# lsl036/STM-Multifrontal-QR-Factorization-Empowered-by-GCN

Hardware: AMD Instinct MI355X
Metric: numerical-factorization GFLOP/s (higher is better)
Workload: dtype f64; 1 GPU; xenon1_colamd_standin: m=49248 n=49248 nnz=1258432 fronts=686 flops/step=5.029e+11, ordering default (COLAMD: qrtest without an ordering argument) (stand-in for xenon1.mtx, absent from the reference checkout); inputs=values resident in HBM, factors left in HBM, parallelism=replica x1, levels=16, retries=0

## Files before the change

stm-multifrontal-qr-factorization-empowered-by-gcn_amd/csrc/stmmqr_kdev.h:

```cpp
#pragma once
#include <hip/hip_runtime.h>
#include <hip/hip_ext.h>
#include <stdint.h>
#include <stdlib.h>
#include "stmmqr_device.h"
#include "stmmqr_kernels.h"
#include "stmmqr_wave.h"
#include "stmmqr_devutil.h"

struct PanelShared {
    double red[16];
    int st_out[STM_NB];
    int dead[STM_NB];
    double nextss;
    int nextss_col;
    int stair[STM_NB];
    int diag[STM_NB];
    double tau[STM_NB];
    double G[STM_NB][STM_NB + 1];
    double T[STM_NB][STM_NB + 1];
    double part[8 * 32];
    double top[2][8];
    double rsum[2][64];
    double rsumB[5][64];
    double Ts[8][9];
    double gp[32];
};

#define NT 256
#define NW (NT / 64)
#define BN 32
#define RB 64
#define VS (RB + 2)
#define WS (BN + 1)

template <int NTH>
__device__ __forceinline__ double block_sum(double v, double *s_red)
{
    v = wave_sum(v);
    __syncthreads();
    if ((threadIdx.x & 63) == 0) s_red[threadIdx.x >> 6] = v;
    __syncthreads();
    double r = 0;
#pragma unroll
    for (int w = 0; w < NTH / 64; w++) r += s_red[w];
    return r;
}

__device__ __forceinline__ int block_incl_scan(int v, int *s_scan, int *total)
{
    const int lane = threadIdx.x & 63, wid = threadIdx.x >> 6;
    int x = v;
#pragma unroll
    for (int o = 1; o < 64; o <<= 1) {
        int y = __shfl_up(x, o, 64);
        if (lane >= o) x += y;
    }
    __syncthreads();
    if (lane == 63) s_scan[wid] = x;
    __syncthreads();
    int base = 0, tot = 0;
#pragma unroll
    for (int w = 0; w < NW; w++) {
        int sw = s_scan[w];
        if (w < wid) base += sw;
        tot += sw;
    }
    *total = tot;
    return x + base;
}

#define SLAB STM_UPD_SLAB
#define CK(x) do { hipError_t e_ = (x); if (e_ != hipSuccess) return (int)e_; } while (0)


struct UpdChunk { double v[8], c[8]; };
__device__ __forceinline__ void upd_chunk_load(UpdChunk &ck, const double *Vg, const double *Cg, long long ld, int i, int mp,
                                               int nbp, int nc, int lcg)
{
    const int ic = min(i, mp - 1);
#pragma unroll
    for (int q = 0; q < 8; q++) {
        const int col = lcg * 8 + q;
        ck.v[q] = Vg[ic + (long long)min(col, nbp - 1) * ld];
        ck.c[q] = Cg[ic + (long long)min(col, nc - 1) * ld];
    }
}
__device__ __forceinline__ void upd_chunk_to_lds(const UpdChunk &ck, int i, int mp, int nbp, int nc, const int *s_pd, int g1,
                                                 int lrow, int lcg, double *Vs, double *Cs, bool c_is_v = false, bool plain = false)
{
    if (plain) {
#pragma unroll
        for (int q = 0; q < 8; q++) {
            const int col = lcg * 8 + q;
            Vs[col * VS + lrow] = ck.v[q];
            Cs[col * VS + lrow] = c_is_v ? ck.v[q] : ck.c[q];
        }
        return;
    }
#pragma unroll
    for (int q = 0; q < 8; q++) {
        const int col = lcg * 8 + q;
        const int d = s_pd[col] - g1;
        const double v = (i < mp && col < nbp && i >= d) ? ((i == d) ? 1.0 : ck.v[q]) : 0.0;
        Vs[col * VS + lrow] = v;
        Cs[col * VS + lrow] = c_is_v ? v : ((i < mp && col < nc) ? ck.c[q] : 0.0);
    }
}

__device__ __forceinline__ void upd_chunk_v_to_lds(const UpdChunk &ck, int i, int mp, int nbp, const int *s_pd, int g1, int lrow,
                                                   int lcg, double *Vs, bool plain = false)
{
    if (plain) {
#pragma unroll
        for (int q = 0; q < 8; q++) Vs[(lcg * 8 + q) * VS + lrow] = ck.v[q];
        return;
    }
#pragma unroll
    for (int q = 0; q < 8; q++) {
        const int col = lcg * 8 + q;
        const int d = s_pd[col] - g1;
        Vs[col * VS + lrow] = (i < mp && col < nbp && i >= d) ? ((i == d) ? 1.0 : ck.v[q]) : 0.0;
    }
}
__device__ __forceinline__ int upd_plain_from(const int *s_pd, int g1, int lane)
{
    const int dm = wave_max_int(lane < STM_NB ? s_pd[lane] : -1);
    return dm >= STM_BIGROW ? STM_BIGROW : dm - g1;
}

__device__ __forceinline__ void dev_T_from_gram(double (*G)[STM_NB + 1], double (*T)[STM_NB + 1], const double *tau, int nc, int tid);

__device__ __forceinline__ d4 dev_w2_tile(const double *Tm, int sq, int sl, const double *W1, int wid, int lane)
{
    const int mi = wid >> 1, ni = wid & 1, l15 = lane & 15, l4 = lane >> 4;
    d4 acc = {0, 0, 0, 0};
    const int nk = mi ? STM_NB / 4 : STM_NB / 8;
#pragma unroll
    for (int kk = 0; kk < STM_NB / 4; kk++) {
        if (kk < nk) {
            const double a = Tm[(4 * kk + l4) * sq + (16 * mi + l15) * sl];
            const double b = W1[(4 * kk + l4) * WS + 16 * ni + l15];
            acc = __builtin_amdgcn_mfma_f64_16x16x4f64(a, b, acc, 0, 0, 0);
        }
    }
    return acc;
}

#define STM_UPD_LDS_DOUBLES (2 * BN * VS + STM_NB * WS)
static_assert(STM_UPD_LDS_DOUBLES == STM_UPD_LDS_HOST, "host sizing of the update kernels' LDS");
template <bool TN = false>
__device__ void dev_update_block(double *F, long long ld, int g1, int mp, int k1, int nbp, const int *diag,
                                 const double *T, int c0, int nc, double *lds, const double *tau = nullptr,
                                 double *Tout = nullptr, double *Tkeep = nullptr)
{
    if (nbp <= 0 || mp <= 0 || nc <= 0) return;
    const int tid = (int)threadIdx.x, lane = tid & 63, wid = tid >> 6;
    const int l15 = lane & 15, l4 = lane >> 4;

    double *Vs = lds;
    double *Cs = Vs + STM_NB * VS;
    double *Ws = Cs + BN * VS;
    __shared__ int s_pd[STM_NB];

    __syncthreads();
    if (tid < STM_NB) s_pd[tid] = (tid < nbp) ? diag[tid] : STM_BIGROW;
    __syncthreads();

    const int lrow = tid & 63, lcg = tid >> 6;
    const double *Vg = F + g1 + (long long)k1 * ld;
    double *Cg = F + g1 + (long long)c0 * ld;

    const int mi = wid >> 1, ni = wid & 1;
    const bool build_t = (tau != nullptr);
    d4 acc = {0, 0, 0, 0}, tot = {0, 0, 0, 0}, gacc = {0, 0, 0, 0}, gtot = {0, 0, 0, 0};
    UpdChunk ck;
    upd_chunk_load(ck, Vg, Cg, ld, lrow, mp, nbp, nc, lcg);
    for (int r0 = 0; r0 < mp; r0 += RB) {
        const int i = r0 + lrow;
        upd_chunk_to_lds(ck, i, mp, nbp, nc, s_pd, g1, lrow, lcg, Vs, Cs);
        __syncthreads();
        if (r0 + RB < mp) upd_chunk_load(ck, Vg, Cg, ld, i + RB, mp, nbp, nc, lcg);
#pragma unroll
        for (int kk = 0; kk < RB / 4; kk++) {
            const double a = Vs[(16 * mi + l15) * VS + 4 * kk + l4];
            const double b = Cs[(16 * ni + l15) * VS + 4 * kk + l4];
            acc = __builtin_amdgcn_mfma_f64_16x16x4f64(a, b, acc, 0, 0, 0);
            if (build_t) {
                const double bv = Vs[(16 * ni + l15) * VS + 4 * kk + l4];
                gacc = __builtin_amdgcn_mfma_f64_16x16x4f64(a, bv, gacc, 0, 0, 0);
            }
        }
        if ((r0 + RB) % STM_UPD_SLAB == 0 || r0 + RB >= mp) {
#pragma unroll
            for (int r = 0; r < 4; r++) { tot[r] += acc[r]; acc[r] = 0; gtot[r] += gacc[r]; gacc[r] = 0; }
        }
        __syncthreads();
    }
#pragma unroll
    for (int r = 0; r < 4; r++) Ws[(16 * mi + l4 + 4 * r) * WS + 16 * ni + l15] = tot[r];
    double *s_Tm = Cs;
    if (build_t) {
        double (*Gm)[STM_NB + 1] = reinterpret_cast<double (*)[STM_NB + 1]>(Vs);
        __shared__ double s_tau_u[STM_NB];
#pragma unroll
        for (int r = 0; r < 4; r++) Gm[16 * mi + l4 + 4 * r][16 * ni + l15] = gtot[r];
        if (tid < STM_NB) s_tau_u[tid] = (tid < nbp) ? tau[tid] : 0.0;
        __syncthreads();
        dev_T_from_gram(Gm, reinterpret_cast<double (*)[STM_NB + 1]>(s_Tm), s_tau_u, nbp, tid);
        if (Tout || Tkeep)
            for (int e = tid; e < STM_NB * STM_NB; e += (int)blockDim.x) {
                const int a = e % STM_NB, b = e / STM_NB;
                const double tv = (a <= b && a < nbp && b < nbp) ? s_Tm[a * WS + b] : 0.0;
                if (Tout) Tout[e] = tv;
                if (Tkeep) Tkeep[e] = tv;
            }
    }
    __syncthreads();

    {
        const int l = tid & 31, cg = tid >> 5;
        double w2[4] = {0, 0, 0, 0};
        if (TN) {
            for (int q = l; q < nbp; q++) {
                const double tq = build_t ? s_Tm[l * WS + q] : T[l + q * STM_NB];
#pragma unroll
                for (int x = 0; x < 4; x++) w2[x] += tq * Ws[q * WS + cg * 4 + x];
            }
            __syncthreads();
#pragma unroll
            for (int x = 0; x < 4; x++) Ws[l * WS + cg * 4 + x] = w2[x];
        } else {
            d4 t2 = {0, 0, 0, 0};
            if (wid < 4) t2 = build_t ? dev_w2_tile(s_Tm, WS, 1, Ws, wid, lane) : dev_w2_tile(T, 1, STM_NB, Ws, wid, lane);
            __syncthreads();
            if (wid < 4) {
#pragma unroll
                for (int r = 0; r < 4; r++) Ws[(16 * mi + l4 + 4 * r) * WS + 16 * ni + l15] = t2[r];
            }
        }
    }
    __syncthreads();

    upd_chunk_load(ck, Vg, Cg, ld, lrow, mp, nbp, nc, lcg);
    for (int r0 = 0; r0 < mp; r0 += RB) {
        const int i = r0 + lrow;
        upd_chunk_to_lds(ck, i, mp, nbp, nc, s_pd, g1, lrow, lcg, Vs, Cs);
        __syncthreads();
        if (r0 + RB < mp) upd_chunk_load(ck, Vg, Cg, ld, i + RB, mp, nbp, nc, lcg);
        d4 u0 = {0, 0, 0, 0}, u1 = {0, 0, 0, 0};
#pragma unroll
        for (int kk = 0; kk < STM_NB / 4; kk++) {
            const double a = Vs[(4 * kk + l4) * VS + 16 * wid + l15];
            const double b0 = Ws[(4 * kk + l4) * WS + l15];
            const double b1 = Ws[(4 * kk + l4) * WS + 16 + l15];
            u0 = __builtin_amdgcn_mfma_f64_16x16x4f64(a, b0, u0, 0, 0, 0);
            u1 = __builtin_amdgcn_mfma_f64_16x16x4f64(a, b1, u1, 0, 0, 0);
        }
#pragma unroll
        for (int r = 0; r < 4; r++) {
            const int row = 16 * wid + l4 + 4 * r;
            Cs[l15 * VS + row] -= u0[r];
            Cs[(16 + l15) * VS + row] -= u1[r];
        }
        __syncthreads();
        if (i < mp) {
#pragma unroll
            for (int q = 0; q < 8; q++) {
                const int col = lcg * 8 + q;
                if (col < nc) Cg[i + col * ld] = Cs[col * VS + lrow];
            }
        }
        __syncthreads();
    }
}

template <int h>
__device__ __forceinline__ void dev_T_merge(double (*G)[STM_NB + 1], double (*T)[STM_NB + 1], int tid)
{
    const int pr = tid / (h * h), ij = tid % (h * h), i = ij / h, j = ij % h;
    const int A0 = 2 * h * pr, B0 = A0 + h;
// ... 142 lines not shown
```

stm-multifrontal-qr-factorization-empowered-by-gcn_amd/csrc/stmmqr_riders.h:

```cpp
#pragma once
#include "stmmqr_kdev.h"


#define STM_PC_LDS_DOUBLES (STM_NB * WS + 4 * BN * VS)
__device__ __forceinline__ void dev_upd_c_h2(const DevCtx &c, const int *__restrict__ flist, const int *__restrict__ plist, int cb0,
                                             const double *Wp, const long long *__restrict__ wpoff, int fi, int cb, int sl0,
                                             int rspw, double *dyn_lds, int *s_pd)
{
    const int f = flist[fi], p = plist[fi];
    const FrontSym s = c.fs[f];
    if (p >= s.npanels) return;
    const PanelDesc *pd = &c.fnum[f].pd[STM_PDI(p)];
    const int g1 = pd->pg1, mp = pd->pt - pd->pg1, nbp = pd->pnb;
    const int nslf = stm_upd_nsl(s);
    const int c0 = pd->pc0 + (cb0 + cb * (1 + c.cbskip)) * BN;
    const int sl = sl0 * rspw, spw = rspw;
    if (nbp <= 0 || mp <= 0 || c0 >= s.fn || sl * SLAB >= mp) return;
    const int nc = min(BN, s.fn - c0);
    const long long ld = s.ld;
    const int half = threadIdx.x >> 8, tid = threadIdx.x & 255, lane = tid & 63, wid = tid >> 6, l15 = lane & 15, l4 = lane >> 4;
    double *Ws = dyn_lds, *Vs = Ws + STM_NB * WS + half * (2 * BN * VS), *Cs = Vs + BN * VS;
    double *s_W1 = dyn_lds + STM_NB * WS, *s_T = s_W1 + BN * VS;
    if (threadIdx.x < STM_NB) s_pd[threadIdx.x] = ((int)threadIdx.x < nbp) ? pd->pdiag[threadIdx.x] : STM_BIGROW;
    const double *Vg = c.Farena + s.foff + g1 + (long long)pd->pk1 * ld;
    double *Cg = c.Farena + s.foff + g1 + (long long)c0 * ld;
    const int lrow = tid & 63, lcg = tid >> 6;
    const int rbeg = sl * SLAB, rend = min(mp, (sl + spw) * SLAB);
    int r0 = rbeg + half * RB;
    UpdChunk ck0, ck1;
    upd_chunk_load(ck0, Vg, Cg, ld, r0 + lrow, mp, nbp, nc, lcg);
    upd_chunk_load(ck1, Vg, Cg, ld, r0 + 2 * RB + lrow, mp, nbp, nc, lcg);
    {
        const double *W0 = Wp + wpoff[fi] + ((long long)cb * nslf) * (STM_NB * BN);
        const double *T = c.Tws + (long long)STM_TSLOT(c.tslot[f], p) * STM_NB * STM_NB;
        for (int e = threadIdx.x; e < STM_NB * BN; e += 2 * NT) {
            const double v = W0[e];
            s_W1[(e / BN) * WS + (e % BN)] = v;
            s_T[(e / STM_NB) * WS + (e % STM_NB)] = T[e];
        }
        __syncthreads();
        d4 w2 = {0, 0, 0, 0};
        if (half == 0) w2 = dev_w2_tile(s_T, 1, WS, s_W1, wid, lane);
        __syncthreads();
        if (half == 0) {
#pragma unroll
            for (int r = 0; r < 4; r++) Ws[(16 * (wid >> 1) + l4 + 4 * r) * WS + 16 * (wid & 1) + l15] = w2[r];
        }
    }
    const int pfrom = upd_plain_from(s_pd, g1, lane);
    const int nch = (rend - rbeg + RB - 1) / RB, trips = (nch + 1) / 2;
    auto trip = [&](UpdChunk &ck) {
        const bool valid = r0 < rend;
        const int i = r0 + lrow;
        double cc[8];
#pragma unroll
        for (int q = 0; q < 8; q++) cc[q] = ck.c[q];
        upd_chunk_v_to_lds(ck, i, mp, nbp, s_pd, g1, lrow, lcg, Vs, valid && r0 > pfrom && r0 + RB <= mp);
        __syncthreads();
        if (r0 + 4 * RB < rend) upd_chunk_load(ck, Vg, Cg, ld, i + 4 * RB, mp, nbp, nc, lcg);
        d4 u0 = {0, 0, 0, 0}, u1 = {0, 0, 0, 0};
#pragma unroll
        for (int kk = 0; kk < STM_NB / 4; kk++) {
            const double a = Vs[(4 * kk + l4) * VS + 16 * wid + l15];
            const double b0 = Ws[(4 * kk + l4) * WS + l15];
            const double b1 = Ws[(4 * kk + l4) * WS + 16 + l15];
            u0 = __builtin_amdgcn_mfma_f64_16x16x4f64(a, b0, u0, 0, 0, 0);
            u1 = __builtin_amdgcn_mfma_f64_16x16x4f64(a, b1, u1, 0, 0, 0);
        }
#pragma unroll
        for (int r = 0; r < 4; r++) {
            const int row = 16 * wid + l4 + 4 * r;
            Cs[l15 * VS + row] = u0[r];
            Cs[(16 + l15) * VS + row] = u1[r];
        }
        __syncthreads();
        if (valid && i < mp) {
#pragma unroll
            for (int q = 0; q < 8; q++) {
                const int col = lcg * 8 + q;
                if (col < nc) Cg[i + col * ld] = cc[q] - Cs[col * VS + lrow];
            }
        }
        r0 += 2 * RB;
    };
    for (int j = 0; j < trips; j += 2) {
        trip(ck0);
        if (j + 1 < trips) trip(ck1);
    }
}
```

stm-multifrontal-qr-factorization-empowered-by-gcn_amd/csrc/stmmqr_update.hip:

```cpp
#include <hip/hip_ext.h>
#include "stmmqr_kdev.h"


__global__ __launch_bounds__(NT) void k_update(DevCtx c, const int *__restrict__ flist, const int *__restrict__ plist, int cb0)
{
    extern __shared__ double dyn_lds[];
    const int f = flist[blockIdx.y];
    const int p = plist[blockIdx.y];
    const FrontSym s = c.fs[f];
    if (p >= s.npanels) return;
    const PanelDesc *pd = &c.fnum[f].pd[STM_PDI(p)];
    const int cbg = cb0 + (int)blockIdx.x * (1 + c.cbskip);
    const int c0 = pd->pc0 + cbg * BN;
    if (c0 >= s.fn) return;
    double *Tw = c.Tws + (long long)STM_TSLOT(c.tslot[f], p) * STM_NB * STM_NB;
    if (pd->t_deferred) {
        const bool first = (cbg == 0) || (c.cbskip > 0 && blockIdx.x == 0);
        dev_update_block(c.Farena + s.foff, s.ld, pd->pg1, pd->pt - pd->pg1, pd->pk1, pd->pnb, pd->pdiag, nullptr, c0,
                         min(BN, s.fn - c0), dyn_lds, c.Tau + s.rp + pd->pk1, first ? Tw : nullptr,
                         (first && c.Tall) ? c.Tall + (long long)(s.tpan + p) * STM_NB * STM_NB : nullptr);
        return;
    }
    dev_update_block(c.Farena + s.foff, s.ld, pd->pg1, pd->pt - pd->pg1, pd->pk1, pd->pnb, pd->pdiag, Tw, c0,
                     min(BN, s.fn - c0), dyn_lds);
// ... 304 lines not shown
            }
            __syncthreads();
        }
    }
    const int nsl = (mp + SLAB - 1) / SLAB;
    const int gslot = (c.ypoff && c.ypoff[f] >= 0) ? min(ncbf, c.sweep) : ncbf;
    double *Wslot = Wp + wpoff[fi] + ((long long)(gram ? gslot : cb) * nslf) * (STM_NB * BN);
    double *W = Wslot + (long long)sl * (STM_NB * BN);
#pragma unroll
    for (int r = 0; r < 4; r++) st_agent(&W[(16 * mi + l4 + 4 * r) * BN + 16 * ni + l15], acc[r]);
    asm volatile("s_waitcnt vmcnt(0)" ::: "memory");
    __syncthreads();
    double *Tslot = c.Tws + (long long)STM_TSLOT(c.tslot[f], p) * STM_NB * STM_NB;
    if (gram) {
        if (tid == 0) {
            s_ticket = __hip_atomic_fetch_add(&num->gcnt, 1, __ATOMIC_RELAXED, __HIP_MEMORY_SCOPE_AGENT);
            if (s_ticket == nsl - 1) {
                __builtin_amdgcn_fence(__ATOMIC_ACQUIRE, "agent");
                asm volatile("s_waitcnt vmcnt(0)" ::: "memory");
                __hip_atomic_store(&num->gcnt, 0, __ATOMIC_RELAXED, __HIP_MEMORY_SCOPE_AGENT);
            }
        }
        __syncthreads();
        if (s_ticket != nsl - 1) return;
        double *s_G = Vs;
        __shared__ double s_tau[STM_NB];
        if (tid < STM_NB) s_tau[tid] = (tid < nbp) ? c.Tau[s.rp + pd->pk1 + tid] : 0.0;
        for (int e = tid; e < STM_NB * BN; e += NT) {
            const double gsum = stm_ordered_sum<true>(Wslot + e, STM_NB * BN, nsl);
            s_G[(e / BN) * WS + (e % BN)] = gsum;
        }
        __syncthreads();
        double *Tkeep = c.Tall ? c.Tall + (long long)(s.tpan + p) * STM_NB * STM_NB : nullptr;
        double (*s_Tb)[STM_NB + 1] = reinterpret_cast<double (*)[STM_NB + 1]>(Cs);
        dev_T_from_gram(reinterpret_cast<double (*)[STM_NB + 1]>(s_G), s_Tb, s_tau, nbp, threadIdx.x);
        for (int e = tid; e < STM_NB * STM_NB; e += NT) {
            const int a = e % STM_NB, b = e / STM_NB;
            const double tv = (a <= b && a < nbp && b < nbp) ? s_Tb[a][b] : 0.0;
            st_agent(&Tslot[e], tv);
            if (Tkeep) Tkeep[e] = tv;
        }
        asm volatile("s_waitcnt vmcnt(0)" ::: "memory");
        __syncthreads();
        if (tid == 0) st_agent(&num->tready, epoch);
        return;
    }
    int *cnt = wcnt + wpoff[fi] / (STM_NB * BN) + cb;
    int *flag = wflag + wpoff[fi] / (STM_NB * BN) + cb;
    bool last = (nsl == 1);
    if (nsl > 1) {
        if (tid == 0) {
            s_ticket = __hip_atomic_fetch_add(cnt, 1, __ATOMIC_RELAXED, __HIP_MEMORY_SCOPE_AGENT);
            if (s_ticket == nsl - 1) {
                __builtin_amdgcn_fence(__ATOMIC_ACQUIRE, "agent");
                asm volatile("s_waitcnt vmcnt(0)" ::: "memory");
                __hip_atomic_store(cnt, 0, __ATOMIC_RELAXED, __HIP_MEMORY_SCOPE_AGENT);
            }
        }
        __syncthreads();
        last = (s_ticket == nsl - 1);
    }
    double *s_W1 = Vs, *s_T = Cs;
    if (last) {
        if (pd->t_deferred && !stm_wait_ge(&num->tready, epoch, c.abort, &s_ok)) { if (tid == 0) STM_SET_PERR(c, num); return; }
        for (int e = tid; e < STM_NB * BN; e += NT) {
            const double v = stm_ordered_sum<true>(Wslot + e, STM_NB * BN, nsl);
            s_W1[(e / BN) * WS + (e % BN)] = v;
            s_T[(e / STM_NB) * WS + (e % STM_NB)] = ld_agent(&Tslot[e]);
        }
        __syncthreads();
        const d4 w2 = dev_w2_tile(s_T, 1, WS, s_W1, wid, lane);
#pragma unroll
        for (int r = 0; r < 4; r++) Ws[(16 * (wid >> 1) + l4 + 4 * r) * WS + 16 * (wid & 1) + l15] = w2[r];
        if (nsl > 1) {
#pragma unroll
            for (int r = 0; r < 4; r++) st_agent(&Wslot[(16 * (wid >> 1) + l4 + 4 * r) * BN + 16 * (wid & 1) + l15], w2[r]);
            asm volatile("s_waitcnt vmcnt(0)" ::: "memory");
            __syncthreads();
            if (tid == 0) st_agent(flag, epoch);
        } else
            __syncthreads();
    } else {
        if (!stm_wait_ge(flag, epoch, c.abort, &s_ok)) { if (tid == 0) STM_SET_PERR(c, num); return; }
        for (int e = tid; e < STM_NB * BN; e += NT) Ws[(e / BN) * WS + (e % BN)] = ld_agent(&Wslot[e]);
        __syncthreads();
    }
#pragma unroll
    for (int q = 0; q < SLAB / RB; q++) {
        const int r0 = r00 + q * RB;
        if (r0 < rend) {
            const int i = r0 + lrow;
            upd_chunk_to_lds(ck[q], i, mp, nbp, nc, s_pd, g1, lrow, lcg, Vs, Cs);
            __syncthreads();
            d4 u0 = {0, 0, 0, 0}, u1 = {0, 0, 0, 0};
#pragma unroll
            for (int kk = 0; kk < STM_NB / 4; kk++) {
                const double a = Vs[(4 * kk + l4) * VS + 16 * wid + l15];
                const double b0 = Ws[(4 * kk + l4) * WS + l15];
                const double b1 = Ws[(4 * kk + l4) * WS + 16 + l15];
                u0 = __builtin_amdgcn_mfma_f64_16x16x4f64(a, b0, u0, 0, 0, 0);
                u1 = __builtin_amdgcn_mfma_f64_16x16x4f64(a, b1, u1, 0, 0, 0);
            }
#pragma unroll
            for (int r = 0; r < 4; r++) {
                const int row = 16 * wid + l4 + 4 * r;
                Cs[l15 * VS + row] -= u0[r];
                Cs[(16 + l15) * VS + row] -= u1[r];
            }
            __syncthreads();
            if (i < mp) {
#pragma unroll
                for (int qq = 0; qq < 8; qq++) {
                    const int col = lcg * 8 + qq;
                    if (col < nc) Cg[i + col * ld] = Cs[col * VS + lrow];
                }
            }
            __syncthreads();
        }
    }
}

__global__ __launch_bounds__(NT, 2) void k_upd_f(DevCtx c, const int *__restrict__ flist, const int *__restrict__ plist, int cb0,
                                              int with_gram, double *Wp, const long long *__restrict__ wpoff, int *wcnt,
                                              int *wflag, int epoch)
{
    extern __shared__ double dyn_lds[];
    dev_k_upd_f(c, flist, plist, cb0, with_gram, Wp, wpoff, wcnt, wflag, epoch, blockIdx.x, blockIdx.y, blockIdx.z, dyn_lds);
}

__device__ __forceinline__ void dev_k_upd_b0(const DevCtx &c, const int *__restrict__ flist, const int *__restrict__ plist, double *Wp,
                                             const long long *__restrict__ wpoff, int *wcnt, int *wflag, int epoch, int sl, int fi,
                                             double *dyn_lds)
{
    __shared__ int s_pd[STM_NB];
    __shared__ int s_ticket, s_ok;
    __shared__ double s_tau[STM_NB];
    const bool tl = (c.dbg & 32768) && c.dbgbuf && threadIdx.x == 0 && sl == 0;
    unsigned long long tl0 = tl ? wall_clock64() : 0;
#define B0TL(k) do { if (tl) { const unsigned long long t1 = wall_clock64(); atomicAdd(&c.dbgbuf[48 + (k)], t1 - tl0); tl0 = t1; } } while (0)
    const int f = flist[fi], p = plist[fi];
    const FrontSym s = c.fs[f];
    if (p >= s.npanels) return;
    FrontNum *num = &c.fnum[f];
    const PanelDesc *pd = &num->pd[STM_PDI(p)];
    const int g1 = pd->pg1, mp = pd->pt - pd->pg1, nbp = pd->pnb;
    const int ncbf = stm_upd_ncb(s, p), nslf = stm_upd_nsl(s);
    if (ncbf <= 0) return;
    const int c0 = pd->pc0;
    if (nbp <= 0 || mp <= 0 || c0 >= s.fn || sl * SLAB >= mp) return;
    const bool deferred = pd->t_deferred != 0;
    const int nc = min(BN, s.fn - c0);
    const long long ld = s.ld;
    const int tid = threadIdx.x, lane = tid & 63, wid = tid >> 6, l15 = lane & 15, l4 = lane >> 4;
    const int lrow = tid & 63, lcg = tid >> 6;
    double *Vs = dyn_lds, *Cs = Vs + STM_NB * VS, *Ws = Cs + BN * VS;
    if (tid < STM_NB) {
        s_pd[tid] = (tid < nbp) ? pd->pdiag[tid] : STM_BIGROW;
        s_tau[tid] = (tid < nbp) ? c.Tau[s.rp + pd->pk1 + tid] : 0.0;
    }
    const double *Vg = c.Farena + s.foff + g1 + (long long)pd->pk1 * ld;
    double *Cg = c.Farena + s.foff + g1 + (long long)c0 * ld;
    const int r00 = sl * SLAB, rend = min(mp, (sl + 1) * SLAB);
    UpdChunk ck[SLAB / RB];
#pragma unroll
    for (int q = 0; q < SLAB / RB; q++) upd_chunk_load(ck[q], Vg, Cg, ld, r00 + q * RB + lrow, mp, nbp, nc, lcg);
    const int nsl = (mp + SLAB - 1) / SLAB;
    const int gslot = (c.ypoff && c.ypoff[f] >= 0) ? min(ncbf, c.sweep) : ncbf;
    double *Wslot = Wp + wpoff[fi];
    double *Gslot = Wp + wpoff[fi] + ((long long)gslot * nslf) * (STM_NB * BN);
    double *Tslot = c.Tws + (long long)STM_TSLOT(c.tslot[f], p) * STM_NB * STM_NB;
    __syncthreads();
    B0TL(0);
    const int mi = wid >> 1, ni = wid & 1;
    d4 acc = {0, 0, 0, 0}, accg = {0, 0, 0, 0};
#pragma unroll
    for (int q = 0; q < SLAB / RB; q++) {
        const int r0 = r00 + q * RB;
        if (r0 < rend) {
            upd_chunk_to_lds(ck[q], r0 + lrow, mp, nbp, nc, s_pd, g1, lrow, lcg, Vs, Cs);
            __syncthreads();
#pragma unroll
            for (int kk = 0; kk < RB / 4; kk++) {
                const double a = Vs[(16 * mi + l15) * VS + 4 * kk + l4];
                const double b = Cs[(16 * ni + l15) * VS + 4 * kk + l4];
                acc = __builtin_amdgcn_mfma_f64_16x16x4f64(a, b, acc, 0, 0, 0);
            }
            if (deferred) {
#pragma unroll
                for (int kk = 0; kk < RB / 4; kk++) {
                    const double a = Vs[(16 * mi + l15) * VS + 4 * kk + l4];
                    const double b = Vs[(16 * ni + l15) * VS + 4 * kk + l4];
                    accg = __builtin_amdgcn_mfma_f64_16x16x4f64(a, b, accg, 0, 0, 0);
                }
            }
            __syncthreads();
        }
    }
    double *s_G = Vs, *s_W1 = Vs + STM_NB * WS, *s_T = Cs;
    B0TL(1);
    bool last = true;
    if (nsl > 1) {
        double *W = Wslot + (long long)sl * (STM_NB * BN), *G = Gslot + (long long)sl * (STM_NB * BN);
#pragma unroll
        for (int r = 0; r < 4; r++) st_agent(&W[(16 * mi + l4 + 4 * r) * BN + 16 * ni + l15], acc[r]);
        if (deferred) {
#pragma unroll
            for (int r = 0; r < 4; r++) st_agent(&G[(16 * mi + l4 + 4 * r) * BN + 16 * ni + l15], accg[r]);
        }
        asm volatile("s_waitcnt vmcnt(0)" ::: "memory");
        __syncthreads();
        int *cnt = wcnt + wpoff[fi] / (STM_NB * BN);
        int *flag = wflag + wpoff[fi] / (STM_NB * BN);
        if (tid == 0) {
            s_ticket = __hip_atomic_fetch_add(cnt, 1, __ATOMIC_RELAXED, __HIP_MEMORY_SCOPE_AGENT);
            if (s_ticket == nsl - 1) {
                __hip_atomic_store(cnt, 0, __ATOMIC_RELAXED, __HIP_MEMORY_SCOPE_AGENT);
                st_agent(flag, epoch);
            }
        }
        __syncthreads();
        last = (s_ticket == nsl - 1);
        B0TL(2);
        if (!stm_wait_ge(flag, epoch, c.abort, &s_ok)) { if (tid == 0) STM_SET_PERR(c, num); return; }
        B0TL(3);
        for (int e = tid; e < STM_NB * BN; e += NT) {
            s_W1[(e / BN) * WS + (e % BN)] = stm_ordered_sum<true>(Wslot + e, STM_NB * BN, nsl);
            if (deferred) s_G[(e / BN) * WS + (e % BN)] = stm_ordered_sum<true>(Gslot + e, STM_NB * BN, nsl);
        }
    } else {
#pragma unroll
        for (int r = 0; r < 4; r++) {
            s_W1[(16 * mi + l4 + 4 * r) * WS + 16 * ni + l15] = acc[r];
            if (deferred) s_G[(16 * mi + l4 + 4 * r) * WS + 16 * ni + l15] = accg[r];
        }
    }
    __syncthreads();
    B0TL(4);
    double (*s_Tb)[STM_NB + 1] = reinterpret_cast<double (*)[STM_NB + 1]>(s_T);
    if (deferred) {
        dev_T_from_gram(reinterpret_cast<double (*)[STM_NB + 1]>(s_G), s_Tb, s_tau, nbp, tid);
        if (last) {
            double *Tkeep = c.Tall ? c.Tall + (long long)(s.tpan + p) * STM_NB * STM_NB : nullptr;
            for (int e = tid; e < STM_NB * STM_NB; e += NT) {
                const int a = e % STM_NB, b = e / STM_NB;
                const double tv = (a <= b && a < nbp && b < nbp) ? s_Tb[a][b] : 0.0;
                Tslot[e] = tv;
                if (Tkeep) Tkeep[e] = tv;
            }
        }
    } else {
        for (int e = tid; e < STM_NB * STM_NB; e += NT) s_Tb[e % STM_NB][e / STM_NB] = Tslot[e];
        __syncthreads();
    }
    B0TL(5);
    {
        const d4 w2 = dev_w2_tile(s_T, WS, 1, s_W1, wid, lane);
#pragma unroll
        for (int r = 0; r < 4; r++) Ws[(16 * (wid >> 1) + l4 + 4 * r) * WS + 16 * (wid & 1) + l15] = w2[r];
    }
    __syncthreads();
    B0TL(6);
#pragma unroll
    for (int q = 0; q < SLAB / RB; q++) {
        const int r0 = r00 + q * RB;
        if (r0 < rend) {
            const int i = r0 + lrow;
            upd_chunk_to_lds(ck[q], i, mp, nbp, nc, s_pd, g1, lrow, lcg, Vs, Cs);
            __syncthreads();
            d4 u0 = {0, 0, 0, 0}, u1 = {0, 0, 0, 0};
#pragma unroll
            for (int kk = 0; kk < STM_NB / 4; kk++) {
                const double a = Vs[(4 * kk + l4) * VS + 16 * wid + l15];
                const double b0 = Ws[(4 * kk + l4) * WS + l15];
                const double b1 = Ws[(4 * kk + l4) * WS + 16 + l15];
                u0 = __builtin_amdgcn_mfma_f64_16x16x4f64(a, b0, u0, 0, 0, 0);
                u1 = __builtin_amdgcn_mfma_f64_16x16x4f64(a, b1, u1, 0, 0, 0);
            }
#pragma unroll
            for (int r = 0; r < 4; r++) {
                const int row = 16 * wid + l4 + 4 * r;
                Cs[l15 * VS + row] -= u0[r];
                Cs[(16 + l15) * VS + row] -= u1[r];
            }
            __syncthreads();
            if (i < mp) {
#pragma unroll
                for (int qq = 0; qq < 8; qq++) {
                    const int col = lcg * 8 + qq;
                    if (col < nc) Cg[i + col * ld] = Cs[col * VS + lrow];
                }
            }
            __syncthreads();
        }
    }
    asm volatile("s_waitcnt vmcnt(0)" ::: "memory");
    B0TL(7);
    if (tl) atomicAdd(&c.dbgbuf[56], 1ull);
#undef B0TL
}

__device__ __forceinline__ void dev_upd_w_rider(const DevCtx &c, const int *__restrict__ flist, const int *__restrict__ plist, int cb0,
                                                double *Wp, const long long *__restrict__ wpoff, int *wcnt, int cb, int y, int rspw,
                                                int fi, double *dyn_lds)
{
    __shared__ int s_pd[STM_NB];
    __shared__ int s_ticket;
    const int f = flist[fi], p = plist[fi];
    const FrontSym s = c.fs[f];
    if (p >= s.npanels) return;
    const PanelDesc *pd = &c.fnum[f].pd[STM_PDI(p)];
    const int g1 = pd->pg1, mp = pd->pt - pd->pg1, nbp = pd->pnb;
    const int ncbf = stm_upd_ncb(s, p), nslf = stm_upd_nsl(s);
    if (cb0 + cb >= ncbf) return;
    const int c0 = pd->pc0 + (cb0 + cb) * BN;
    const int sl0 = y * rspw;
    if (nbp <= 0 || mp <= 0 || c0 >= s.fn || sl0 * SLAB >= mp) return;
    const int nc = min(BN, s.fn - c0);
    const long long ld = s.ld;
    const int tid = threadIdx.x, lane = tid & 63, wid = tid >> 6, l15 = lane & 15, l4 = lane >> 4;
    double *Vs = dyn_lds, *Cs = Vs + STM_NB * VS;
    if (tid < STM_NB) s_pd[tid] = (tid < nbp) ? pd->pdiag[tid] : STM_BIGROW;
    __syncthreads();
    const double *Vg = c.Farena + s.foff + g1 + (long long)pd->pk1 * ld;
    const double *Cg = c.Farena + s.foff + g1 + (long long)c0 * ld;
    const int mi = wid >> 1, ni = wid & 1;
    const int nsl = (mp + SLAB - 1) / SLAB;
    const int rend = min(mp, (sl0 + rspw) * SLAB);
    double *W = Wp + wpoff[fi] + ((long long)cb * nslf + sl0) * (STM_NB * BN);
    d4 acc = {0, 0, 0, 0};
    UpdChunk ck;
    upd_chunk_load(ck, Vg, Cg, ld, sl0 * SLAB + (tid & 63), mp, nbp, nc, tid >> 6);
    const int pfrom = (nc == BN) ? upd_plain_from(s_pd, g1, lane) : STM_BIGROW;
    int done = 0;
    for (int r0 = sl0 * SLAB; r0 < rend; r0 += RB) {
        upd_chunk_to_lds(ck, r0 + (tid & 63), mp, nbp, nc, s_pd, g1, tid & 63, tid >> 6, Vs, Cs, false, r0 > pfrom && r0 + RB <= mp);
        __syncthreads();
        if (r0 + RB < rend) upd_chunk_load(ck, Vg, Cg, ld, r0 + RB + (tid & 63), mp, nbp, nc, tid >> 6);
#pragma unroll
        for (int kk = 0; kk < RB / 4; kk++) {
            const double a = Vs[(16 * mi + l15) * VS + 4 * kk + l4];
            const double b = Cs[(16 * ni + l15) * VS + 4 * kk + l4];
            acc = __builtin_amdgcn_mfma_f64_16x16x4f64(a, b, acc, 0, 0, 0);
        }
        __syncthreads();
        if (((r0 + RB) % SLAB) == 0 || r0 + RB >= rend) {
            if (nsl == 1) {
#pragma unroll
                for (int r = 0; r < 4; r++) W[(16 * mi + l4 + 4 * r) * BN + 16 * ni + l15] = acc[r];
            } else {
#pragma unroll
                for (int r = 0; r < 4; r++) st_agent(&W[(16 * mi + l4 + 4 * r) * BN + 16 * ni + l15], acc[r]);
            }
            W += STM_NB * BN;
            acc = d4{0, 0, 0, 0};
            done++;
        }
    }
    if (nsl == 1) return;
    asm volatile("s_waitcnt vmcnt(0)" ::: "memory");
    __syncthreads();
    int *cnt = wcnt + wpoff[fi] / (STM_NB * BN) + cb;
    if (tid == 0) {
        s_ticket = __hip_atomic_fetch_add(cnt, done, __ATOMIC_RELAXED, __HIP_MEMORY_SCOPE_AGENT);
        if (s_ticket + done == nsl) {
            __builtin_amdgcn_fence(__ATOMIC_ACQUIRE, "agent");
            asm volatile("s_waitcnt vmcnt(0)" ::: "memory");
            __hip_atomic_store(cnt, 0, __ATOMIC_RELAXED, __HIP_MEMORY_SCOPE_AGENT);
        }
    }
    __syncthreads();
    if (s_ticket + done != nsl) return;
    double *W0 = Wp + wpoff[fi] + ((long long)cb * nslf) * (STM_NB * BN);
    double v[STM_NB * BN / NT];
#pragma unroll
    for (int q = 0; q < STM_NB * BN / NT; q++) v[q] = stm_ordered_sum<true>(W0 + tid + q * NT, STM_NB * BN, nsl);
#pragma unroll
    for (int q = 0; q < STM_NB * BN / NT; q++) W0[tid + q * NT] = v[q];
}

__global__ __launch_bounds__(NT, 2) void k_upd_b0w(DevCtx c, const int *__restrict__ flist, const int *__restrict__ plist, int nfr,
                                                   int maxsl, int ncbrest, double *Wp, const long long *__restrict__ wpoff, int *wcnt,
                                                   int *wflag, int epoch, double *Wp2, int *wcnt2, int rspw)
{
    extern __shared__ double dyn_lds[];
    if ((int)blockIdx.z < nfr) {
        if ((int)blockIdx.x >= maxsl || blockIdx.y >= 1) return;
        dev_k_upd_b0(c, flist, plist, Wp, wpoff, wcnt, wflag, epoch, blockIdx.x, blockIdx.z, dyn_lds);
        return;
    }
    if ((int)blockIdx.x >= ncbrest || (int)blockIdx.y * rspw >= maxsl) return;
    dev_upd_w_rider(c, flist, plist, 1, Wp2, wpoff, wcnt2, blockIdx.x, blockIdx.y, rspw, (int)blockIdx.z - nfr, dyn_lds);
}

__global__ __launch_bounds__(NT, 2) void k_upd_fw(DevCtx c, const int *__restrict__ flist, const int *__restrict__ plist, int nfr,
                                                  int maxsl, int ncbrest, double *Wp, const long long *__restrict__ wpoff, int *wcnt,
                                                  int *wflag, int epoch, double *Wp2, int *wcnt2)
{
    extern __shared__ double dyn_lds[];
    if ((int)blockIdx.z < nfr) {
        if ((int)blockIdx.x >= maxsl || blockIdx.y >= 2) return;
        dev_k_upd_f(c, flist, plist, 0, 1, Wp, wpoff, wcnt, wflag, epoch, blockIdx.x, blockIdx.y, blockIdx.z, dyn_lds);
        return;
    }
    if ((int)blockIdx.x >= ncbrest || (int)blockIdx.y >= maxsl) return;
    dev_k_upd_w<true>(c, flist, plist, 1, 0, Wp2, wpoff, wcnt2, blockIdx.x, blockIdx.y, (int)blockIdx.z - nfr, ncbrest, dyn_lds);
}
int stm_update_lds_bytes(void) { return (int)((2 * BN * VS + STM_NB * WS) * sizeof(double)); }
int stm_launch_update(const DevCtx &c, const int *flist, const int *plist, int nfr, int cb0, int ncb, hipStream_t st)
{
    if (nfr <= 0 || ncb <= 0) return 0;
    hipLaunchKernelGGL(k_update, dim3(ncb, nfr), dim3(NT), (size_t)stm_update_lds_bytes(), st, c, flist, plist, cb0);
    return (int)hipGetLastError();
}
int stm_launch_update_split(const DevCtx &c, const int *flist, const int *plist, int nfr, int cb0, int ncb, int maxsl, double *Wp,
                            const long long *wpoff, int *wcnt, int with_gram, hipStream_t st)
{
    if (nfr <= 0 || ncb + (with_gram ? 1 : 0) <= 0 || maxsl <= 0) return 0;
    const size_t lds = (size_t)stm_update_lds_bytes();
    hipLaunchKernelGGL(k_upd_w, dim3(ncb + (with_gram ? 1 : 0), maxsl, nfr), dim3(NT), (size_t)(2 * BN * VS) * sizeof(double), st, c,
                       flist, plist, cb0, with_gram ? 1 : 0, Wp, wpoff, wcnt);
    if (ncb > 0) hipLaunchKernelGGL(k_upd_c, dim3(ncb, maxsl, nfr), dim3(NT), lds, st, c, flist, plist, cb0, (const double *)Wp, wpoff);
    return (int)hipGetLastError();
}
int stm_launch_update_fused(const DevCtx &c, const int *flist, const int *plist, int nfr, int cb0, int ncb, int maxsl, double *Wp,
                            const long long *wpoff, int *wcnt, int *wflag, int epoch, int with_gram, hipStream_t st)
{
    const int ny = ncb + (with_gram ? 1 : 0);
    if (nfr <= 0 || ny <= 0 || maxsl <= 0) return 0;
    hipLaunchKernelGGL(k_upd_f, dim3(maxsl, ny, nfr), dim3(NT), (size_t)stm_update_lds_bytes(), st, c, flist, plist, cb0,
                       with_gram ? 1 : 0, Wp, wpoff, wcnt, wflag, epoch);
    return (int)hipGetLastError();
}
int stm_launch_update_fw(const DevCtx &c, const int *flist, const int *plist, int nfr, int ncb, int maxsl, double *Wp,
                         const long long *wpoff, int *wcnt, int *wflag, int epoch, double *Wp2, int *wcnt2, hipStream_t st)
{
    if (nfr <= 0 || maxsl <= 0) return 0;
    const int rest = ncb - 1;
    static int one = -1;
    if (one < 0) one = getenv("STMMQR_B0_ONE") ? atoi(getenv("STMMQR_B0_ONE")) : 1;
    if (one) {
        static int rspw = -1;
        if (rspw < 0) rspw = getenv("STMMQR_RSPW_W") && atoi(getenv("STMMQR_RSPW_W")) > 0 ? atoi(getenv("STMMQR_RSPW_W")) : 2;
        const int uy = (maxsl + rspw - 1) / rspw;
        hipLaunchKernelGGL(k_upd_b0w, dim3(maxsl > rest ? maxsl : rest, rest > 0 ? uy : 1, rest > 0 ? 2 * nfr : nfr), dim3(NT),
                           (size_t)stm_update_lds_bytes(), st, c, flist, plist, nfr, maxsl, rest > 0 ? rest : 0, Wp, wpoff, wcnt, wflag, epoch,
                           Wp2, wcnt2, rspw);
        return (int)hipGetLastError();
    }
// ... 52 lines not shown
```

Measured before the change: 5512 GFLOP/s.

## Apply trailing update per wave from registers, removing LDS staging and barriers

Restructures the C -= V*W update so each wave owns 16-row tiles whose V and C values are loaded straight into MFMA operand registers. W is held in registers per wave, so the per-chunk LDS staging of V and C and the block-wide barriers around it are no longer needed. The rider kernel now streams tiles with a three-buffer register prefetch across all waves. The fused update kernel's epilogue also applies directly from registers. The cost is more register pressure and less coalesced global loads, since each lane now reads strided columns.

New measurement: 5610 GFLOP/s (median of 6 runs). 1.02x the previous value.

```diff
diff --git a/stm-multifrontal-qr-factorization-empowered-by-gcn_amd/csrc/stmmqr_kdev.h b/stm-multifrontal-qr-factorization-empowered-by-gcn_amd/csrc/stmmqr_kdev.h
--- a/stm-multifrontal-qr-factorization-empowered-by-gcn_amd/csrc/stmmqr_kdev.h
+++ b/stm-multifrontal-qr-factorization-empowered-by-gcn_amd/csrc/stmmqr_kdev.h
@@ -127,6 +127,106 @@
 {
     const int dm = wave_max_int(lane < STM_NB ? s_pd[lane] : -1);
     return dm >= STM_BIGROW ? STM_BIGROW : dm - g1;
+}
+
+struct UpdTile { double v[8], c[8]; };
+__device__ __forceinline__ void upd_tile_load(UpdTile &t, const double *Vg, const double *Cg, long long ld, int i, int mp, int nbp,
+                                              int nc, int l4)
+{
+    const int ic = min(i, mp - 1);
+#pragma unroll
+    for (int q = 0; q < 8; q++) {
+        t.v[q] = Vg[ic + (long long)min(4 * q + l4, nbp - 1) * ld];
+        t.c[q] = Cg[ic + (long long)min(16 * (q >> 2) + l4 + 4 * (q & 3), nc - 1) * ld];
+    }
+}
+__device__ __forceinline__ void upd_tile_vmask(double (&vm)[8], const UpdTile &t, int i, int mp, int nbp, const int *s_pd, int g1,
+                                               int l4, bool plain = false)
+{
+#pragma unroll
+    for (int q = 0; q < 8; q++) {
+        const int col = 4 * q + l4;
+        const int d = plain ? -1 : s_pd[col] - g1;
+        vm[q] = plain ? t.v[q] : ((i < mp && col < nbp && i >= d) ? ((i == d) ? 1.0 : t.v[q]) : 0.0);
+    }
+}
+__device__ __forceinline__ void upd_tile_to_lds(const UpdTile &t, int i, int mp, int nbp, int nc, const int *s_pd, int g1, int lrow,
+                                                int l4, double *Vs, double *Cs)
+{
+    double vm[8];
+    upd_tile_vmask(vm, t, i, mp, nbp, s_pd, g1, l4);
+#pragma unroll
+    for (int q = 0; q < 8; q++) {
+        const int col = 16 * (q >> 2) + l4 + 4 * (q & 3);
+        Vs[(4 * q + l4) * VS + lrow] = vm[q];
+        Cs[col * VS + lrow] = (i < mp && col < nc) ? t.c[q] : 0.0;
+    }
+}
+struct UpdTileW { double a0[8], a1[8]; };
+__device__ __forceinline__ void upd_tile_w(UpdTileW &w, const double *Ws, int l15, int l4)
+{
+#pragma unroll
+    for (int q = 0; q < 8; q++) {
+        w.a0[q] = Ws[(4 * q + l4) * WS + l15];
+        w.a1[q] = Ws[(4 * q + l4) * WS + 16 + l15];
+    }
+}
+__device__ __forceinline__ void upd_tile_apply(const double (&vm)[8], const UpdTile &t, const UpdTileW &w, double *Cg, long long ld,
+                                               int i, int mp, int nc, int l4)
+{
+    d4 u0 = {0, 0, 0, 0}, u1 = {0, 0, 0, 0};
+#pragma unroll
+    for (int kk = 0; kk < STM_NB / 4; kk++) {
+        u0 = __builtin_amdgcn_mfma_f64_16x16x4f64(w.a0[kk], vm[kk], u0, 0, 0, 0);
+        u1 = __builtin_amdgcn_mfma_f64_16x16x4f64(w.a1[kk], vm[kk], u1, 0, 0, 0);
+    }
+    if (i < mp) {
+#pragma unroll
+        for (int r = 0; r < 4; r++) {
+            const int col = l4 + 4 * r;
+            if (col < nc) Cg[i + (long long)col * ld] = t.c[r] - u0[r];
+            if (16 + col < nc) Cg[i + (long long)(16 + col) * ld] = t.c[4 + r] - u1[r];
+        }
+    }
+}
+
+#ifndef UPD_TILE_RUN
+#define UPD_TILE_RUN 1
+#endif
+template <int NWV>
+__device__ __forceinline__ int upd_tile_of(int wv, int n)
+{
+    return UPD_TILE_RUN * (wv + NWV * (n / UPD_TILE_RUN)) + n % UPD_TILE_RUN;
+}
+template <int NWV>
+__device__ __forceinline__ void upd_tile_stream_first(UpdTile &tb0, UpdTile &tb1, const double *Vg, const double *Cg, long long ld, int rbeg,
+                                                      int wv, int l15, int l4, int mp, int nbp, int nc)
+{
+    upd_tile_load(tb0, Vg, Cg, ld, rbeg + 16 * upd_tile_of<NWV>(wv, 0) + l15, mp, nbp, nc, l4);
+    upd_tile_load(tb1, Vg, Cg, ld, rbeg + 16 * upd_tile_of<NWV>(wv, 1) + l15, mp, nbp, nc, l4);
+}
+template <int NWV>
+__device__ __forceinline__ void upd_tile_stream(UpdTile &tb0, UpdTile &tb1, const UpdTileW &w, const double *Vg, double *Cg, long long ld,
+                                                int rbeg, int rend, int wv, int l15, int l4, int mp, int nbp, int nc, const int *s_pd,
+                                                int g1, int pfrom)
+{
+    const int ntile = (rend - rbeg + 15) >> 4;
+    int n = 0;
+    UpdTile tb2;
+    auto step = [&](UpdTile &cur, UpdTile &nxt) {
+        const int r0 = rbeg + 16 * upd_tile_of<NWV>(wv, n), i = r0 + l15;
+        double vm[8];
+        upd_tile_vmask(vm, cur, i, mp, nbp, s_pd, g1, l4, r0 > pfrom && r0 + 16 <= mp);
+        const int t2 = upd_tile_of<NWV>(wv, n + 2);
+        if (t2 < ntile) upd_tile_load(nxt, Vg, Cg, ld, rbeg + 16 * t2 + l15, mp, nbp, nc, l4);
+        upd_tile_apply(vm, cur, w, Cg, ld, i, rend, nc, l4);
+        n++;
+    };
+    while (upd_tile_of<NWV>(wv, n) < ntile) {
+        step(tb0, tb2);
+        if (upd_tile_of<NWV>(wv, n) < ntile) step(tb1, tb0);
+        if (upd_tile_of<NWV>(wv, n) < ntile) step(tb2, tb1);
+    }
 }
 
 __device__ __forceinline__ void dev_T_from_gram(double (*G)[STM_NB + 1], double (*T)[STM_NB + 1], const double *tau, int nc, int tid);
diff --git a/stm-multifrontal-qr-factorization-empowered-by-gcn_amd/csrc/stmmqr_riders.h b/stm-multifrontal-qr-factorization-empowered-by-gcn_amd/csrc/stmmqr_riders.h
--- a/stm-multifrontal-qr-factorization-empowered-by-gcn_amd/csrc/stmmqr_riders.h
+++ b/stm-multifrontal-qr-factorization-empowered-by-gcn_amd/csrc/stmmqr_riders.h
@@ -2,7 +2,7 @@
 #include "stmmqr_kdev.h"
 
 
-#define STM_PC_LDS_DOUBLES (STM_NB * WS + 4 * BN * VS)
+#define STM_PC_LDS_DOUBLES (3 * STM_NB * WS)
 __device__ __forceinline__ void dev_upd_c_h2(const DevCtx &c, const int *__restrict__ flist, const int *__restrict__ plist, int cb0,
                                              const double *Wp, const long long *__restrict__ wpoff, int fi, int cb, int sl0,
                                              int rspw, double *dyn_lds, int *s_pd)
@@ -18,18 +18,16 @@
     if (nbp <= 0 || mp <= 0 || c0 >= s.fn || sl * SLAB >= mp) return;
     const int nc = min(BN, s.fn - c0);
     const long long ld = s.ld;
-    const int half = threadIdx.x >> 8, tid = threadIdx.x & 255, lane = tid & 63, wid = tid >> 6, l15 = lane & 15, l4 = lane >> 4;
-    double *Ws = dyn_lds, *Vs = Ws + STM_NB * WS + half * (2 * BN * VS), *Cs = Vs + BN * VS;
-    double *s_W1 = dyn_lds + STM_NB * WS, *s_T = s_W1 + BN * VS;
+    const int lane = threadIdx.x & 63, wv = threadIdx.x >> 6, l15 = lane & 15, l4 = lane >> 4;
+    double *Ws = dyn_lds, *s_W1 = Ws + STM_NB * WS, *s_T = s_W1 + STM_NB * WS;
     if (threadIdx.x < STM_NB) s_pd[threadIdx.x] = ((int)threadIdx.x < nbp) ? pd->pdiag[threadIdx.x] : STM_BIGROW;
     const double *Vg = c.Farena + s.foff + g1 + (long long)pd->pk1 * ld;
     double *Cg = c.Farena + s.foff + g1 + (long long)c0 * ld;
-    const int lrow = tid & 63, lcg = tid >> 6;
     const int rbeg = sl * SLAB, rend = min(mp, (sl + spw) * SLAB);
-    int r0 = rbeg + half * RB;
-    UpdChunk ck0, ck1;
-    upd_chunk_load(ck0, Vg, Cg, ld, r0 + lrow, mp, nbp, nc, lcg);
-    upd_chunk_load(ck1, Vg, Cg, ld, r0 + 2 * RB + lrow, mp, nbp, nc, lcg);
+    constexpr int NWV = 2 * NT / 64;
+    UpdTile tb0, tb1;
+    upd_tile_stream_first<NWV>(tb0, tb1, Vg, Cg, ld, rbeg, wv, l15, l4, mp, nbp, nc);
+    UpdTileW w;
     {
         const double *W0 = Wp + wpoff[fi] + ((long long)cb * nslf) * (STM_NB * BN);
         const double *T = c.Tws + (long long)STM_TSLOT(c.tslot[f], p) * STM_NB * STM_NB;
@@ -39,52 +37,13 @@
             s_T[(e / STM_NB) * WS + (e % STM_NB)] = T[e];
         }
         __syncthreads();
-        d4 w2 = {0, 0, 0, 0};
-        if (half == 0) w2 = dev_w2_tile(s_T, 1, WS, s_W1, wid, lane);
-        __syncthreads();
-        if (half == 0) {
+        if (wv < 4) {
+            const d4 w2 = dev_w2_tile(s_T, 1, WS, s_W1, wv, lane);
 #pragma unroll
-            for (int r = 0; r < 4; r++) Ws[(16 * (wid >> 1) + l4 + 4 * r) * WS + 16 * (wid & 1) + l15] = w2[r];
-        }
-    }
-    const int pfrom = upd_plain_from(s_pd, g1, lane);
-    const int nch = (rend - rbeg + RB - 1) / RB, trips = (nch + 1) / 2;
-    auto trip = [&](UpdChunk &ck) {
-        const bool valid = r0 < rend;
-        const int i = r0 + lrow;
-        double cc[8];
-#pragma unroll
-        for (int q = 0; q < 8; q++) cc[q] = ck.c[q];
-        upd_chunk_v_to_lds(ck, i, mp, nbp, s_pd, g1, lrow, lcg, Vs, valid && r0 > pfrom && r0 + RB <= mp);
-        __syncthreads();
-        if (r0 + 4 * RB < rend) upd_chunk_load(ck, Vg, Cg, ld, i + 4 * RB, mp, nbp, nc, lcg);
-        d4 u0 = {0, 0, 0, 0}, u1 = {0, 0, 0, 0};
-#pragma unroll
-        for (int kk = 0; kk < STM_NB / 4; kk++) {
-            const double a = Vs[(4 * kk + l4) * VS + 16 * wid + l15];
-            const double b0 = Ws[(4 * kk + l4) * WS + l15];
-            const double b1 = Ws[(4 * kk + l4) * WS + 16 + l15];
-            u0 = __builtin_amdgcn_mfma_f64_16x16x4f64(a, b0, u0, 0, 0, 0);
-            u1 = __builtin_amdgcn_mfma_f64_16x16x4f64(a, b1, u1, 0, 0, 0);
-        }
-#pragma unroll
-        for (int r = 0; r < 4; r++) {
-            const int row = 16 * wid + l4 + 4 * r;
-            Cs[l15 * VS + row] = u0[r];
-            Cs[(16 + l15) * VS + row] = u1[r];
+            for (int r = 0; r < 4; r++) Ws[(16 * (wv >> 1) + l4 + 4 * r) * WS + 16 * (wv & 1) + l15] = w2[r];
         }
         __syncthreads();
-        if (valid && i < mp) {
-#pragma unroll
-            for (int q = 0; q < 8; q++) {
-                const int col = lcg * 8 + q;
-                if (col < nc) Cg[i + col * ld] = cc[q] - Cs[col * VS + lrow];
-            }
-        }
-        r0 += 2 * RB;
-    };
-    for (int j = 0; j < trips; j += 2) {
-        trip(ck0);
-        if (j + 1 < trips) trip(ck1);
+        upd_tile_w(w, Ws, l15, l4);
     }
+    upd_tile_stream<NWV>(tb0, tb1, w, Vg, Cg, ld, rbeg, rend, wv, l15, l4, mp, nbp, nc, s_pd, g1, upd_plain_from(s_pd, g1, lane));
 }
diff --git a/stm-multifrontal-qr-factorization-empowered-by-gcn_amd/csrc/stmmqr_update.hip b/stm-multifrontal-qr-factorization-empowered-by-gcn_amd/csrc/stmmqr_update.hip
--- a/stm-multifrontal-qr-factorization-empowered-by-gcn_amd/csrc/stmmqr_update.hip
+++ b/stm-multifrontal-qr-factorization-empowered-by-gcn_amd/csrc/stmmqr_update.hip
@@ -480,7 +480,7 @@
     const int nc = min(BN, s.fn - c0);
     const long long ld = s.ld;
     const int tid = threadIdx.x, lane = tid & 63, wid = tid >> 6, l15 = lane & 15, l4 = lane >> 4;
-    const int lrow = tid & 63, lcg = tid >> 6;
+    const int lrow = 16 * wid + l15;
     double *Vs = dyn_lds, *Cs = Vs + STM_NB * VS, *Ws = Cs + BN * VS;
     if (tid < STM_NB) {
         s_pd[tid] = (tid < nbp) ? pd->pdiag[tid] : STM_BIGROW;
@@ -489,9 +489,9 @@
     const double *Vg = c.Farena + s.foff + g1 + (long long)pd->pk1 * ld;
     double *Cg = c.Farena + s.foff + g1 + (long long)c0 * ld;
     const int r00 = sl * SLAB, rend = min(mp, (sl + 1) * SLAB);
-    UpdChunk ck[SLAB / RB];
-#pragma unroll
-    for (int q = 0; q < SLAB / RB; q++) upd_chunk_load(ck[q], Vg, Cg, ld, r00 + q * RB + lrow, mp, nbp, nc, lcg);
+    UpdTile ck[SLAB / RB];
+#pragma unroll
+    for (int q = 0; q < SLAB / RB; q++) upd_tile_load(ck[q], Vg, Cg, ld, r00 + q * RB + lrow, mp, nbp, nc, l4);
     const int nsl = (mp + SLAB - 1) / SLAB;
     const int gslot = (c.ypoff && c.ypoff[f] >= 0) ? min(ncbf, c.sweep) : ncbf;
     double *Wslot = Wp + wpoff[fi];
@@ -505,7 +505,7 @@
     for (int q = 0; q < SLAB / RB; q++) {
         const int r0 = r00 + q * RB;
         if (r0 < rend) {
-            upd_chunk_to_lds(ck[q], r0 + lrow, mp, nbp, nc, s_pd, g1, lrow, lcg, Vs, Cs);
+            upd_tile_to_lds(ck[q], r0 + lrow, mp, nbp, nc, s_pd, g1, lrow, l4, Vs, Cs);
             __syncthreads();
 #pragma unroll
             for (int kk = 0; kk < RB / 4; kk++) {
@@ -588,40 +588,20 @@
     }
     __syncthreads();
     B0TL(6);
-#pragma unroll
-    for (int q = 0; q < SLAB / RB; q++) {
-        const int r0 = r00 + q * RB;
-        if (r0 < rend) {
-            const int i = r0 + lrow;
-            upd_chunk_to_lds(ck[q], i, mp, nbp, nc, s_pd, g1, lrow, lcg, Vs, Cs);
-            __syncthreads();
-            d4 u0 = {0, 0, 0, 0}, u1 = {0, 0, 0, 0};
-#pragma unroll
-            for (int kk = 0; kk < STM_NB / 4; kk++) {
-                const double a = Vs[(4 * kk + l4) * VS + 16 * wid + l15];
-                const double b0 = Ws[(4 * kk + l4) * WS + l15];
-                const double b1 = Ws[(4 * kk + l4) * WS + 16 + l15];
-                u0 = __builtin_amdgcn_mfma_f64_16x16x4f64(a, b0, u0, 0, 0, 0);
-                u1 = __builtin_amdgcn_mfma_f64_16x16x4f64(a, b1, u1, 0, 0, 0);
-            }
-#pragma unroll
-            for (int r = 0; r < 4; r++) {
-                const int row = 16 * wid + l4 + 4 * r;
-                Cs[l15 * VS + row] -= u0[r];
-                Cs[(16 + l15) * VS + row] -= u1[r];
-            }
-            __syncthreads();
-            if (i < mp) {
-#pragma unroll
-                for (int qq = 0; qq < 8; qq++) {
-                    const int col = lcg * 8 + qq;
-                    if (col < nc) Cg[i + col * ld] = Cs[col * VS + lrow];
-                }
-            }
-            __syncthreads();
-        }
-    }
-    asm volatile("s_waitcnt vmcnt(0)" ::: "memory");
+    {
+        UpdTileW w;
+        upd_tile_w(w, Ws, l15, l4);
+#pragma unroll
+        for (int q = 0; q < SLAB / RB; q++) {
+            const int r0 = r00 + q * RB;
+            if (r0 < rend) {
+                const int i = r0 + lrow;
+                double vm[8];
+                upd_tile_vmask(vm, ck[q], i, mp, nbp, s_pd, g1, l4);
+                upd_tile_apply(vm, ck[q], w, Cg, ld, i, mp, nc, l4);
+            }
+        }
+    }
     B0TL(7);
     if (tl) atomicAdd(&c.dbgbuf[56], 1ull);
 #undef B0TL
```
